# 0xPARC/plonkathon

Measured on AMD Instinct MI355X. Metric: proofs/sec at group_order=2^11 (PLONK prover hot path: NTT + quotient + KZG MSM), higher is better.
Workload: dtype u32x8 (254-bit Montgomery integers, BN254 Fr/Fq); 1 GPU; configs[1]: group_order=2^11, powersOfTau28_hez_final_11 SRS slice, synthetic squaring-chain witness, one distinct witness per proof; lockstep_batch=512, streams_per_gpu=20, parallelism=proof-sharded x1, ranks_in_communicator=1, gather_transport=none (single rank), msm_table_bytes=157571612672

## Files before the change

### plonkathon_amd/csrc/hip_compat.h

```cpp
#pragma once
#ifdef PLONK_EMU
#include "hip_emu.h"
#else
#include <hip/hip_runtime.h>
#define PLONK_HD __host__ __device__ __forceinline__
#define PLONK_HD_NOINLINE __host__ __device__ inline __attribute__((noinline))
#ifdef PLONK_FP_OUTLINE
#define PLONK_FP_CALL __host__ __device__ __attribute__((noinline))
#else
#define PLONK_FP_CALL __host__ __device__ __forceinline__
#endif
#define PLONK_DEV __device__ __forceinline__
#define PLONK_LAMBDA_INLINE __attribute__((always_inline))
#define PLONK_KERNEL(...) HIP_KERNEL_NAME(__VA_ARGS__)
#define PLONK_LAUNCH(kern, grid, block, shmem, stream, ...) \
    hipLaunchKernelGGL(kern, grid, block, shmem, stream, __VA_ARGS__)
#ifdef __HIP_DEVICE_COMPILE__
#define PLONK_SCHED_FENCE() __builtin_amdgcn_sched_barrier(0)
#else
#define PLONK_SCHED_FENCE() ((void)0)
#endif
#define PLONK_DYN_SMEM(name) extern __shared__ __attribute__((aligned(16))) unsigned char name[]
#endif

#ifndef PLONK_SHORT_KERNEL_PRIORITY
#define PLONK_SHORT_KERNEL_PRIORITY 3
#endif
#ifndef PLONK_WORK_KERNEL_PRIORITY
#define PLONK_WORK_KERNEL_PRIORITY 1
#endif
#if defined(__HIP_DEVICE_COMPILE__)
#define PLONK_SHORT_KERNEL() __builtin_amdgcn_s_setprio(PLONK_SHORT_KERNEL_PRIORITY)
#define PLONK_WORK_KERNEL() __builtin_amdgcn_s_setprio(PLONK_WORK_KERNEL_PRIORITY)
#else
#define PLONK_SHORT_KERNEL() ((void)0)
#define PLONK_WORK_KERNEL() ((void)0)
#endif

#ifndef PLONK_SMALL_FORMS
#define PLONK_SMALL_FORMS 23
#endif
#define PLONK_BESIDE_ACC(lanes, bit) PLONK_BESIDE_ACC_##bit(lanes)
#if (PLONK_SMALL_FORMS) & 1
#define PLONK_BESIDE_ACC_1(lanes) __launch_bounds__(lanes, 5)
#else
#define PLONK_BESIDE_ACC_1(lanes) __launch_bounds__(lanes)
#endif
#if (PLONK_SMALL_FORMS) & 2
#define PLONK_BESIDE_ACC_2(lanes) __launch_bounds__(lanes, 5)
#else
#define PLONK_BESIDE_ACC_2(lanes) __launch_bounds__(lanes)
#endif
#if (PLONK_SMALL_FORMS) & 4
#define PLONK_BESIDE_ACC_4(lanes) __launch_bounds__(lanes, 5)
#else
#define PLONK_BESIDE_ACC_4(lanes) __launch_bounds__(lanes)
#endif
#if (PLONK_SMALL_FORMS) & 16
#define PLONK_BESIDE_ACC_16(lanes) __launch_bounds__(lanes, 5)
#else
#define PLONK_BESIDE_ACC_16(lanes) __launch_bounds__(lanes)
#endif

#if defined(__HIP_DEVICE_COMPILE__)
#define PLONK_CHAIN_BEGIN() uint32_t plonk_chain_tok = 0
#define PLONK_CHAIN(acc) asm("" : "=s"(plonk_chain_tok) : "v"(acc), "0"(plonk_chain_tok))
#define PLONK_CHAIN_END(word) asm("" : "+v"(word) : "s"(plonk_chain_tok))
#else
#define PLONK_CHAIN_BEGIN() ((void)0)
#define PLONK_CHAIN(acc) ((void)0)
#define PLONK_CHAIN_END(word) ((void)0)
#endif
```

### plonkathon_amd/csrc/msm_comb.h

```cpp
#pragma once
#include <utility>

#include "msm_common.h"

#define MSM_COMB_MAX_TEETH 24
#define MSM_COMB_SEG_BITS 8
#define MSM_COMB_SCALAR_BITS 254
#define MSM_COMB_REDO 0x80000000u
PLONK_HD bool msm_comb_needs_redo(uint32_t v) { return (v & MSM_COMB_REDO) != 0 || v > MSM_DEFER_CAP; }

#define MSM_COMB_SKIP 0xffffffffu
struct alignas(16) MsmCombDigit4 { uint32_t d[4]; };

PLONK_HD unsigned msm_comb_columns(unsigned h) { return (MSM_COMB_SCALAR_BITS + h - 1) / h; }

struct MsmCombShape {
    unsigned h, a;
    unsigned top_bits, top_g;
    unsigned top_b;
    uint32_t top_entries;
};
PLONK_HD constexpr MsmCombShape msm_comb_shape(unsigned h, bool top) {
    MsmCombShape s{h, (MSM_COMB_SCALAR_BITS + h - 1) / h, 0, 0, 0, 0};
    if (!top) return s;
// ... 466 lines not shown
    ok &= g1l_wave_reduce_step<2>(acc, lane);
    ok &= g1l_wave_reduce_step<1>(acc, lane);
    if (!ok) atomicOr(n_deferred + m, MSM_COMB_REDO);
    if (lane == 0) colsum[m * a + j] = g1l_to_piece_wide(acc);
}

template <unsigned LPM> __global__ void PLONK_BESIDE_ACC(64, 1) msm_comb_finalize_kernel(const G1Xyzz* sums, size_t M, unsigned G, unsigned a,
                                                                                       const G1Affine* lookup, unsigned hb, size_t n,
                                                                                       const MsmDeferred* deferred, size_t deferred_stride,
                                                                                       uint32_t* n_deferred, uint32_t* redo, Fq* out_xy, uint8_t* flags,
                                                                                       unsigned n_real, unsigned top_delta) {
    PLONK_SHORT_KERNEL();
    const size_t gid = (size_t)blockIdx.x * 64 + threadIdx.x, m = gid / LPM;
    const unsigned l = (unsigned)(gid % LPM), lane = threadIdx.x;
    G1XyzzL acc = g1l_identity();
    bool ok = true;
    bool listed = false;
    if (m < M && l < a) {
        const uint32_t seen = n_deferred[m];
        listed = l == 0 && msm_comb_needs_redo(seen);
        const uint32_t nd = msm_comb_needs_redo(seen) ? 0u : seen;
        const unsigned jtop = l + ((a - 1 - l) / LPM) * LPM;
#pragma unroll 1
        for (int j = (int)jtop; j >= 0; j -= (int)LPM) {
            if (j != (int)jtop)
#pragma unroll 1
                for (unsigned d = 0; d < LPM; d++) g1l_dbl(acc);
#pragma unroll 1
            for (unsigned g = 0; g < G; g++) ok &= g1l_add_fast<true>(acc, g1l_from_piece(&sums[(m * G + g) * a + j]));
#pragma unroll 1
            for (uint32_t k = 0; k < nd; k++) {
                const MsmDeferred e = deferred[m * deferred_stride + k];
                if (e.bucket / n != (uint32_t)j || e.entry == MSM_COMB_SKIP) continue;
                const size_t i = e.bucket - (size_t)j * n;
                const G1Affine* src = lookup + ((msm_comb_block_of(i, n_real, top_delta) << hb) + (e.entry & 0x7fffffffu));
                const Fq x = fp_load(&src->x), y = fp_load(&src->y);
                if (!(fp_is_zero(x) && fp_is_zero(y))) ok &= g1l_madd_fast(acc, x, y, (e.entry >> 31) != 0);
            }
        }
#pragma unroll 1
        for (unsigned d = 0; d < l; d++) g1l_dbl(acc);
    }
    if constexpr (LPM >= 2) ok &= g1l_wave_reduce_step<1, true>(acc, lane);
    if constexpr (LPM >= 4) ok &= g1l_wave_reduce_step<2, true>(acc, lane);
    if constexpr (LPM >= 8) ok &= g1l_wave_reduce_step<4, true>(acc, lane);
    if constexpr (LPM >= 16) ok &= g1l_wave_reduce_step<8, true>(acc, lane);
    if constexpr (LPM >= 32) ok &= g1l_wave_reduce_step<16, true>(acc, lane);
    if constexpr (LPM >= 64) ok &= g1l_wave_reduce_step<32, true>(acc, lane);
    if (m < M && !ok && !msm_comb_needs_redo(atomicOr(n_deferred + m, MSM_COMB_REDO))) listed = true;
    if (listed) msm_redo_append(redo, (uint32_t)m, (uint32_t)M);
    if (m < M && l == 0) msm_store_result(g1l_to_xyzz(acc), m, out_xy, flags);
}

__global__ void __launch_bounds__(256) msm_comb_slow_kernel(const G1Affine* lookup, unsigned hb, unsigned a, const uint32_t* digits, size_t n, size_t rs,
                                                            size_t is, const uint32_t* redo, unsigned M, Fq* out_xy, uint8_t* flags, unsigned n_real,
                                                            unsigned top_delta) {
    PLONK_SHORT_KERNEL();
    __shared__ G1Xyzz red[256];
    const unsigned tid = threadIdx.x, count = redo[0] < M ? redo[0] : M;
#pragma unroll 1
    for (unsigned k = blockIdx.x; k < count; k += gridDim.x) {
        const unsigned m = redo[1 + k];
        if (m >= M) continue;
        const uint32_t* dg = digits + (size_t)m * a * rs;
        G1Xyzz acc = g1_xyzz_identity();
#pragma unroll 1
        for (int j = (int)a - 1; j >= 0; j--) {
            g1_dbl(acc);
#pragma unroll 1
            for (size_t i = tid; i < n; i += 256) {
                const uint32_t d = dg[(size_t)j * rs + i * is];
                if (d == MSM_COMB_SKIP) continue;
                const G1Affine* src = lookup + ((msm_comb_block_of(i, n_real, top_delta) << hb) + (d & 0x7fffffffu));
                G1Affine pt;
                pt.x = fp_load(&src->x);
                pt.y = fp_load(&src->y);
                if (d >> 31) pt.y = fp_neg(pt.y);
                g1_madd<true>(acc, pt);
            }
        }
        msm_fold_store(red, acc, tid, 256, m, out_xy, flags);
        __syncthreads();
    }
}

PLONK_DEV bool msm_comb_entry_matches(const G1Affine& P0, const MsmCombScale& k, unsigned a, unsigned h, uint32_t idx, const G1Affine* e) {
    const G1Affine P = g1_to_affine(msm_comb_scaled_base(P0, k));
    const G1Xyzz v = msm_comb_entry_slow(P, a, h, idx);
    const Fq ex = fp_load(&e->x), ey = fp_load(&e->y);
    if (g1_is_identity(v)) return fp_is_zero(ex) && fp_is_zero(ey);
    return fp_eq(fp_mul(ex, v.zz), v.x) && fp_eq(fp_mul(ey, v.zzz), v.y);
}
__global__ void __launch_bounds__(64) msm_comb_verify_kernel(const G1Affine* bases, const G1Affine* lookup, size_t n, unsigned a, unsigned h,
                                                             unsigned samples, MsmCombScale k, unsigned* mismatches) {
    const size_t t = (size_t)blockIdx.x * blockDim.x + threadIdx.x;
    if (t >= n + 2 * (size_t)samples) return;
    const uint32_t mask = (1u << (h - 1)) - 1u;
    size_t i;
    uint32_t idx;
    if (t < n) {
        i = t;
        idx = mask;
    } else {
        const unsigned s = (unsigned)(t - n) >> 1;
        i = n <= samples ? (s < n ? s : n - 1) : (size_t)s * (n - 1) / (samples - 1);
        idx = ((t - n) & 1) ? (0x55555555u & mask) : 0u;
    }
    G1Affine b;
    b.x = fp_load(&bases[i].x);
    b.y = fp_load(&bases[i].y);
    if (!msm_comb_entry_matches(b, k, a, h, idx, lookup + ((i << (h - 1)) + idx))) atomicAdd(mismatches, 1u);
}

__global__ void __launch_bounds__(64) msm_comb_verify_top_kernel(const G1Affine* bases, const G1Affine* lookup, size_t n, unsigned a, unsigned h, unsigned g,
                                                                 unsigned B, MsmCombScale k, unsigned* mismatches) {
    const size_t grp = (size_t)blockIdx.x * blockDim.x + threadIdx.x;
    if (grp >= msm_comb_top_groups(n, g)) return;
    const unsigned L = a * h, j = (unsigned)(grp % a);
    G1Xyzz sum = g1_xyzz_identity();
    uint32_t idx = 0, pw = 1;
#pragma unroll 1
    for (unsigned pos = 0; pos < g; pos++, pw *= B) {
        const size_t i = grp * g + pos;
        idx += ((B - 1) / 2 + (i < n ? 1u : 0u)) * pw;
        if (i >= n) continue;
        G1Affine b;
        b.x = fp_load(&bases[i].x);
        b.y = fp_load(&bases[i].y);
        G1Xyzz p = msm_comb_scaled_base(b, k);
#pragma unroll 1
        for (unsigned d = 0; d < L - j; d++) g1_dbl(p);
// ... 237 lines not shown
```

### plonkathon_amd/csrc/prover.hip

```cpp
#include <assert.h>
#include <string.h>

#include <array>
#include <vector>

#include "prover.h"
#include "g1_codec.h"
#include "prover_scans.h"
#include "prover_intake.h"
#include "prover_blind.h"

__global__ void pi_coeffs_kernel(const Fr* pub, size_t l, const Fr* roots_inv, size_t n, size_t B, Fr n_inv, Fr* pic) {
    PLONK_SHORT_KERNEL();
    const size_t total = B * n;
    for (size_t gI = (size_t)blockIdx.x * blockDim.x + threadIdx.x; gI < total; gI += (size_t)gridDim.x * blockDim.x) {
        const size_t b = gI / n, j = gI - b * n;
        Fr acc = fp_zero<FrParams>();
        for (size_t i = 0; i < l; i++) acc = fp_add(acc, fp_mul(fp_load(pub + b * l + i), fp_load(roots_inv + ((i * j) & (n - 1)))));
        fp_store(pic + gI, fp_neg(fp_mul(acc, n_inv)));
    }
}
__global__ void pi_coset_kernel(const Fr* pub, size_t l, const Fr* li_big, size_t n4, size_t B, Fr* pi_big) {
    PLONK_SHORT_KERNEL();
    const size_t total = B * n4;
    for (size_t gI = (size_t)blockIdx.x * blockDim.x + threadIdx.x; gI < total; gI += (size_t)gridDim.x * blockDim.x) {
        const size_t b = gI / n4, k = gI - b * n4;
        Fr acc = fp_zero<FrParams>();
        for (size_t i = 0; i < l; i++) acc = fp_add(acc, fp_mul(fp_load(pub + b * l + i), fp_load(li_big + i * n4 + k)));
        fp_store(pi_big + gI, fp_neg(acc));
    }
}
struct Zh4 { Fr v[4]; };
__global__ void li_coset_kernel(const Fr* xs, const Fr* roots, size_t n4, size_t n, size_t l, Zh4 zh, Fr n_inv, Fr* li) {
    const size_t total = l * n4;
    for (size_t gI = (size_t)blockIdx.x * blockDim.x + threadIdx.x; gI < total; gI += (size_t)gridDim.x * blockDim.x) {
        const size_t i = gI / n4, k = gI - i * n4;
        const Fr wi = fp_load(roots + i);
        const Fr num = fp_mul(fp_mul(wi, n_inv), zh.v[k / n]);
        fp_store(li + gI, fp_mul(num, fp_inv(fp_sub(fp_load(xs + k), wi))));
    }
}

__global__ void __launch_bounds__(2 * TC_LANES) transcript_kernel(int round, ProofState* st, size_t B, const Fq* commit_xy,
                                                                  const uint8_t* flags, ChallengeConsts cc) {
    PLONK_SHORT_KERNEL();
    __shared__ TcShared shared[2];
    const unsigned grp = threadIdx.x / TC_LANES, lane = threadIdx.x % TC_LANES;
    TcShared& sh = shared[grp];
    size_t b = (size_t)blockIdx.x * 2 + grp;
    const bool live = b < B;
    if (!live) b = B - 1;
    ProofState& s = st[b];
    TcState t = tc_load(s.transcript, lane);
    uint32_t error = 0;
    Fr c0 = fp_zero<FrParams>(), c1 = fp_zero<FrParams>();

    if (round >= 1 && round <= 3) {
        const unsigned first_slot = round == 1 ? 0 : round == 2 ? 3 : 4, count = round == 2 ? 1 : 3;
        if (lane < 2 * count) {
            const size_t slot = (size_t)first_slot + lane / 2;
            const uint8_t fl = flags[slot * B + b];
            Fq v = fp_load(commit_xy + 2 * (slot * B + b) + (lane & 1));
            if (fl) {
                v = fp_zero<FqParams>();
                error = 1;
            }
            limbs_to_be32(v.v, sh.msg + 32 * lane);
        }
    } else if (round == 4 && lane < PROOF_EVALS) {
        Fr e = fp_from_mont(s.evals[lane]);
        limbs_to_be32(e.v, sh.msg + 32 * lane);
    }
    __syncthreads();
    tc_round(t, sh, lane, cc, round, c0, c1);
    if (!live) return;
    tc_store(t, lane, s.transcript);
    if (error) s.error = 1;
    if (lane == 0) {
        if (round == 0) s.error = 0;
        if (round == 1) { s.beta = c0; s.gamma = c1; }
        if (round == 2) { s.alpha = c0; s.fft_cofactor = c1; }
        if (round == 3) s.zeta = c0;
        if (round == 4) s.v = c0;
    }
}

struct ZhInv { Fr v[4]; };
struct QuotientIn { const Fr* wit[5]; const Fr* fixed[FX_COUNT]; const Fr* l0; const Fr* xs; const uint32_t* cid; unsigned fixed_stride; };
__global__ void __launch_bounds__(256) quotient_kernel(QuotientIn in, ZhInv zh, const ProofState* st, RoundChallenges direct, unsigned n4, Fr* quot,
                                                       unsigned coset_log, unsigned out_stride) {
    PLONK_WORK_KERNEL();
    typedef FpL<FrParams> L;
    const unsigned b = blockIdx.y;
    const L beta = fpl_from_fp_uniform(st ? st[b].beta : direct.beta), gamma = fpl_from_fp_uniform(st ? st[b].gamma : direct.gamma),
            alpha = fpl_from_fp_uniform(st ? st[b].alpha : direct.alpha);
    const L one = fpl_one<FrParams>();
    const size_t row = (size_t)b * n4;
    const size_t fx = in.cid ? (size_t)in.cid[b] * in.fixed_stride : 0;
    for (unsigned k = blockIdx.x * blockDim.x + threadIdx.x; k < n4; k += gridDim.x * blockDim.x) {
        const unsigned cr = coset_log ? k >> coset_log : 0u, cmask = coset_log ? (1u << coset_log) - 1u : 0u;
        const unsigned kw = coset_log ? ((k & ~cmask) | ((k + 1) & cmask))
                                      : ((k + 4 < n4) ? k + 4 : k + 4 - n4);
        const auto ld = [&](const Fr* p) PLONK_LAMBDA_INLINE { return fpl_from_fp(fp_load(p)); };
        const L a = ld(in.wit[0] + row + k), bb = ld(in.wit[1] + row + k), c = ld(in.wit[2] + row + k);
        const L t1 = fpl_mul_add(a, ld(in.fixed[FX_QL] + fx + k), bb, ld(in.fixed[FX_QR] + fx + k));
        const L ab = fpl_mul(a, bb);
        const L t2 = fpl_mul_add(ab, ld(in.fixed[FX_QM] + fx + k), c, ld(in.fixed[FX_QO] + fx + k));
        const L gate = fpl_norm(fpl_add(fpl_add(t1, t2), fpl_add(ld(in.wit[3] + row + k), ld(in.fixed[FX_QC] + fx + k))));
        const L bx = fpl_mul(beta, ld(in.xs + k));
        const L u1 = fpl_norm(fpl_add(gamma, bx));
        const L u2 = fpl_norm(fpl_add(u1, bx));
        const L u3 = fpl_norm(fpl_add(u2, bx));
        const L z = ld(in.wit[4] + row + k);
        L p1 = fpl_mul(fpl_add(a, u1), z);
        p1 = fpl_mul(fpl_add(bb, u2), p1);
        p1 = fpl_mul(fpl_add(c, u3), p1);
        const L v1 = fpl_norm(fpl_add(gamma, fpl_mul(beta, ld(in.fixed[FX_S1] + fx + k))));
        L p2 = fpl_mul(fpl_add(a, v1), ld(in.wit[4] + row + kw));
        const L v2 = fpl_norm(fpl_add(gamma, fpl_mul(beta, ld(in.fixed[FX_S2] + fx + k))));
        p2 = fpl_mul(fpl_add(bb, v2), p2);
        const L v3 = fpl_norm(fpl_add(gamma, fpl_mul(beta, ld(in.fixed[FX_S3] + fx + k))));
        p2 = fpl_mul(fpl_add(c, v3), p2);
        const L first = fpl_mul(fpl_sub(z, one), ld(in.l0 + k));
        const L inner = fpl_add(fpl_sub(p1, p2), fpl_mul(alpha, first));
        const L acc = fpl_add(gate, fpl_mul(alpha, inner));
        L zhi;
        if (coset_log >= 6) zhi = fpl_from_fp_uniform(zh.v[cr]);
        else zhi = fpl_from_fp(zh.v[coset_log ? cr : (k & 3)]);
        fp_store(quot + (size_t)b * out_stride + k, fpl_pack_canonical(fpl_mul(acc, zhi)));
    }
}

__global__ void quotient_combine_kernel(Fr* quot, size_t n, size_t stride, size_t B, Fr ci, Fr g1_inv, Fr g2_inv_half, Fr half) {
    PLONK_SHORT_KERNEL();
    const size_t total = B * n;
    for (size_t gI = (size_t)blockIdx.x * blockDim.x + threadIdx.x; gI < total; gI += (size_t)gridDim.x * blockDim.x) {
        const size_t b = gI / n, i = gI - b * n;
        Fr* q = quot + b * stride + i;
        const Fr h0 = fp_load(q), h1 = fp_load(q + n), h2 = fp_load(q + 2 * n);
        const Fr s1 = fp_sub(h0, h2), p = fp_add(h0, h2);
        const Fr m = fp_sub(fp_dbl(h1), fp_mul(ci, s1));
        fp_store(q, fp_mul(fp_add(p, m), half));
// ... 161 lines not shown
static size_t batch_n_vectors(const plonk_prover* p) { return 17 + 5 * p->circuit.qcosets; }
static std::array<BatchBuffer, 14> batch_buffers(plonk_prover* p) {
    plonk_prover::Rounds& r = p->rounds;
    plonk_prover::Results& o = p->results;
    const size_t e = sizeof(Fr);
    return {{{(void**)&r.wit_lag, STAGED_N_VECTORS, 0, 0, true}, {(void**)&r.z_lag, 1}, {(void**)&r.coef, 5}, {(void**)&r.big, 5 * p->circuit.qcosets}, {(void**)&r.quot, 4},
             {(void**)&r.num, 1}, {(void**)&r.wz, 2}, {(void**)&r.closes, 0, 2 * sizeof(uint32_t)}, {(void**)&r.lin_w, 0, sizeof(LinWeights)}, {(void**)&r.blind, 0, sizeof(BlindState)},
             {(void**)&o.commit_xy, 0, PROOF_POINTS * 2 * sizeof(Fq)}, {(void**)&o.commit_flags, 0, PROOF_POINTS},
             {(void**)&o.state, 0, sizeof(ProofState)}, {(void**)&p->intake.pub, 0, p->circuit.n_public * e, e, true}}};
}

static void free_batch(plonk_prover* p, bool rounds_only = false) {
    for (const BatchBuffer& b : batch_buffers(p))
        if (!(rounds_only && b.in_set)) dev_free_all({b.slot});
    dev_free_all({(void**)&p->rounds.seg});
    p->rounds.seg_cap = p->intake.resident_b = p->rounds.cap_b = 0;
    if (rounds_only) return;
    dev_free_all({(void**)&p->intake.vars.buf});
    p->intake.vars.cap = p->intake.cap_b = 0;
}

static int ensure_segments(plonk_prover* p, size_t B) {
    const size_t need = scan_scratch_elems(B, prover_segments(p, B));
    return dev_grow(p->circuit.ctx->stream, &p->rounds.seg_cap, need, {{(void**)&p->rounds.seg, need * sizeof(Fr)}});
}

static int ensure_buffers(plonk_prover* p, size_t B, bool rounds_only) {
    if (B <= p->rounds.cap_b && (rounds_only || B <= p->intake.cap_b)) return ensure_segments(p, B);
    PLONK_CHECK_HIP(hipStreamSynchronize(p->circuit.ctx->stream));
    free_batch(p, rounds_only);
    int rc = PLONK_OK;
    size_t vectors = 0;
    for (const BatchBuffer& b : batch_buffers(p)) {
        if (rc == PLONK_OK && !(rounds_only && b.in_set)) rc = dev_alloc(b.slot, B * (b.n_vectors * p->circuit.n * sizeof(Fr) + b.bytes) + b.extra);
        vectors += b.n_vectors;
    }
    assert(vectors == batch_n_vectors(p));
    if (rc != PLONK_OK) {
        free_batch(p, rounds_only);
        if (rc == PLONK_ERR_NOMEM)
            plonk_set_error("a batch of %zu proofs of group_order %zu needs %zu bytes of device memory", B, p->circuit.n,
                            batch_n_vectors(p) * B * p->circuit.n * sizeof(Fr));
        return rc;
    }
    p->rounds.cap_b = B;
    if (!rounds_only) p->intake.cap_b = B;
    return ensure_segments(p, B);
}
static int ensure_batch(plonk_prover* p, size_t B) { return ensure_buffers(p, B, false); }
static int ensure_rounds(plonk_prover* p, size_t B) { return ensure_buffers(p, B, true); }

static void transcript_round(plonk_prover* p, size_t B, int round) {
    PLONK_LAUNCH(transcript_kernel, dim3((unsigned)((B + 1) / 2)), dim3(2 * TC_LANES), 0, p->circuit.ctx->stream, round, p->results.state, B,
                 (const Fq*)p->results.commit_xy, (const uint8_t*)p->results.commit_flags, p->circuit.chal);
}

static int commit(plonk_prover* p, size_t B, const Fr* lag, const Fr* coef, size_t count, size_t first_point) {
    const plonk_prover::Circuit& c = p->circuit;
    return msm_run_device(c.ctx, p->lag_srs ? p->lag_srs : c.srs, p->lag_srs ? lag : coef, c.n, count * B, c.n, p->results.commit_xy + 2 * first_point * B,
                          p->results.commit_flags + first_point * B);
}

static void blind_commit(plonk_prover* p, size_t B, unsigned first_point, unsigned count) {
    PLONK_LAUNCH(blind_commit_kernel, dim3((unsigned)B, count), dim3(BLIND_LANES), 0, p->circuit.ctx->stream, (const BlindState*)p->rounds.blind,
                 (const G1Affine*)p->blinding_src.htab, first_point, B, p->results.commit_xy, p->results.commit_flags);
}

static int blinders_for_run(plonk_prover* p, size_t B) {
    plonk_prover::Blinding& bl = p->blinding_src;
    hipStream_t s = p->circuit.ctx->stream;
    PLONK_REQUIRE(!bl.explicit_batch || bl.explicit_batch == B, PLONK_ERR_STATE, "run: batch %zu, but the blinders were set for a batch of %zu", B,
                  bl.explicit_batch);
    PLONK_REQUIRE(bl.explicit_batch || bl.seeded, PLONK_ERR_STATE,
                  "run: batch %zu is to be blinded, but neither plonk_prover_set_blinders nor plonk_prover_seed_blinders has been called", B);
    if (bl.explicit_batch) {
        PLONK_LAUNCH(blind_load_kernel, grid1(B * BLIND_COUNT), dim3(256), 0, s, (const Fr*)bl.explicit_b, B, p->rounds.blind);
        bl.explicit_batch = 0;
    } else {
        BlindSeed in;
        memcpy(in.seed, bl.seed, 32);
        in.run = bl.runs;
        PLONK_LAUNCH(blind_derive_kernel, dim3((unsigned)((B + 1) / 2)), dim3(2 * TC_LANES), 0, s, in, B, p->circuit.chal, p->rounds.blind);
    }
    bl.runs++;
    return PLONK_OK;
}

static int prover_init(plonk_prover* p, plonk_ctx* ctx, plonk_srs* srs, unsigned log_n, unsigned K, const uint8_t* selectors_le32, const size_t* n_public);

static int prover_create(plonk_ctx* ctx, plonk_srs* srs, unsigned log_n, unsigned K, const uint8_t* selectors_le32, const size_t* n_public, plonk_prover** out) {
    PLONK_ENTER(ctx);
    PLONK_REQUIRE(log_n >= 1 && log_n + 2 <= PLONK_FR_TWO_ADICITY, PLONK_ERR_ARG, "group_order 2^%u out of range", log_n);
    const size_t n = (size_t)1 << log_n;
    PLONK_REQUIRE(log_n <= PROVER_MAX_LOG_N, PLONK_ERR_ARG, "the batched prover supports group_order <= %u (got %zu)", 1u << PROVER_MAX_LOG_N, n);
    PLONK_REQUIRE(srs->n_points >= n, PLONK_ERR_ARG, "SRS has %zu powers, group_order is %zu", srs->n_points, n);
    for (unsigned c = 0; c < K; c++) PLONK_REQUIRE(n_public[c] <= n, PLONK_ERR_ARG, "more public inputs than rows");
    plonk_prover* p = new plonk_prover();
    memset((void*)p, 0, sizeof *p);
    const int rc = prover_init(p, ctx, srs, log_n, K, selectors_le32, n_public);
    if (rc != PLONK_OK) {
        plonk_prover_destroy(p);
        return rc;
    }
    *out = p;
    return PLONK_OK;
}

// ... 144 lines not shown
    PLONK_ENTER(p->circuit.ctx);
    const unsigned seg = (flags & PLONK_PROVER_SEGMENTS_MASK) >> 8;
    PLONK_REQUIRE(seg <= 9 && (!seg || (p->circuit.n >> (seg - 1)) >= 16), PLONK_ERR_ARG,
                  "2^%u segments: at most 256, of at least 16 rows each (group_order %zu)", seg ? seg - 1 : 0, p->circuit.n);
    const unsigned form = (flags & PLONK_PROVER_SOLVE_FORM_MASK) >> 16;
    PLONK_REQUIRE(form <= PLONK_PROVER_SOLVE_LEVELS, PLONK_ERR_ARG, "solve form %u: 0 (automatic), 1 (one lane per proof) or 2 (levels)", form);
    const bool blinding = (flags & PLONK_PROVER_BLINDING) != 0;
    if (blinding != p->blinding) PLONK_TRY(set_blinding(p, blinding));
    p->seg_forced = seg;
    p->solve_forced = form;
    p->lag_srs = nullptr;
    if (flags & PLONK_PROVER_LAGRANGE_COMMITS) PLONK_TRY(msm_lagrange_srs(p->circuit.ctx, p->circuit.srs, p->circuit.log_n, &p->lag_srs));
    return PLONK_OK;
}

int plonk_prover_destroy(plonk_prover* p) {
    if (!p) return PLONK_OK;
    plonk_prover::Circuit& c = p->circuit;
    if (c.ctx) {
        plonk_use_device(c.ctx->device);
        hipStreamSynchronize(c.ctx->stream);
        if (c.ctx->copy_stream) hipStreamSynchronize(c.ctx->copy_stream);
    }
    free_batch(p);
    free_coset_tables(c);
    dev_free_all({(void**)&c.fixed_lag, (void**)&c.fixed_coef, (void**)&p->blinding_src.htab, (void**)&p->blinding_src.explicit_b});
    intake_destroy(p);
    free(c.n_public_of);
    delete p;
    return PLONK_OK;
}

int plonk_prover_run(plonk_prover* p, size_t B) {
    PLONK_REQUIRE(p && B, PLONK_ERR_ARG, "bad argument");
    PLONK_REQUIRE(B == p->intake.resident_b, PLONK_ERR_STATE, "run: batch %zu, but %zu witnesses are resident", B, p->intake.resident_b);
    const plonk_prover::Circuit& c = p->circuit;
    const plonk_prover::Rounds& r = p->rounds;
    PLONK_ENTER(c.ctx);
    plonk_ctx* ctx = c.ctx;
    const size_t n = c.n, n4 = 4 * n;
    const unsigned log_n = c.log_n;
    hipStream_t s = ctx->stream;
    const Fr* pub = p->intake.pub;
    ProofState* state = p->results.state;
    PLONK_REQUIRE(B <= 65535, PLONK_ERR_ARG, "batch %zu exceeds 65535 (the proofs are a grid's second dimension)", B);
    PLONK_TRY(ensure_segments(p, B));
    const unsigned S = prover_segments(p, B);
    const bool blind = p->blinding;
    BlindState* bs = r.blind;
    if (blind) PLONK_TRY(blinders_for_run(p, B));
    const uint32_t* cid = c.n_circuits > 1 ? p->labels.dev : nullptr;

    transcript_round(p, B, 0);
    PLONK_CHECK_HIP(hipMemsetAsync(r.closes + B, 0, B * sizeof(uint32_t), s));
    PLONK_LAUNCH(gate_check_kernel, grid1(B * n), dim3(256), 0, s, (const Fr*)r.wit_lag, pub, c.n_public,
                 c.sparse_pi ? (const Fr*)nullptr : (const Fr*)(r.wit_lag + 3 * B * n), (const Fr*)c.fixed_lag, cid, n, B, r.closes + B);
    if (c.sparse_pi) {
        PLONK_TRY(ntt_run(ctx, ntt_inverse(r.wit_lag, r.coef, log_n, 3 * B)));
        if (c.n_public) PLONK_LAUNCH(pi_coeffs_kernel, grid1(B * n), dim3(256), 0, s, pub, c.n_public, c.roots_inv, n, B, c.n_inv, r.coef + 3 * B * n);
        else PLONK_CHECK_HIP(hipMemsetAsync(r.coef + 3 * B * n, 0, B * n * sizeof(Fr), s));
    } else {
        PLONK_TRY(ntt_run(ctx, ntt_inverse(r.wit_lag, r.coef, log_n, 4 * B)));
    }
    PLONK_TRY(commit(p, B, r.wit_lag, r.coef, 3, 0));
    if (blind) blind_commit(p, B, 0, 3);
    transcript_round(p, B, 1);
    GrandProductIn gp = {};
    for (int k = 0; k < 3; k++) {
        gp.abc[k] = r.wit_lag + (size_t)k * B * n;
        gp.sig[k] = c.fixed_lag + (FX_S1 + k) * n;
    }
    gp.cid = cid;
    gp.sig_stride = FX_COUNT * n;
    PLONK_TRY(prof_begin(ctx, "prover_grand_product", 11.0 * 32.0 * (double)n * (double)B));
    PLONK_TRY(scan_grand_product(s, S, gp, c.roots, state, RoundChallenges{}, n, B, r.z_lag, r.closes, r.num, r.wz, r.seg));
    PLONK_TRY(prof_end(ctx));
    PLONK_TRY(ntt_run(ctx, ntt_inverse(r.z_lag, r.coef + 4 * B * n, log_n, B)));
    PLONK_TRY(commit(p, B, r.z_lag, r.coef + 4 * B * n, 1, 3));
    if (blind) blind_commit(p, B, 3, 1);
    transcript_round(p, B, 2);
    const size_t n3 = c.qcosets * n;
    if (c.sparse_pi) {
        PLONK_TRY(ntt_run(ctx, coset_call(c, r.coef, r.big, 3 * B)));
        PLONK_TRY(ntt_run(ctx, coset_call(c, r.coef + 4 * B * n, r.big + 4 * B * n3, B)));
        if (c.n_public) PLONK_LAUNCH(pi_coset_kernel, grid1(B * n3), dim3(256), 0, s, pub, c.n_public, (const Fr*)c.li_big, n3, B, r.big + 3 * B * n3);
        else PLONK_CHECK_HIP(hipMemsetAsync(r.big + 3 * B * n3, 0, B * n3 * sizeof(Fr), s));
    } else {
        PLONK_TRY(ntt_run(ctx, coset_call(c, r.coef, r.big, 5 * B)));
    }
    if (blind) {
        BlindZh bz;
        for (int k = 0; k < 4; k++) bz.v[k] = c.zh[k];
        PLONK_LAUNCH(blind_coset_kernel, grid1(B * n3), dim3(256), 0, s, (const BlindState*)bs, (const Fr*)c.x_big, bz, log_n, B, r.big);
    }
    ZhInv zh;
    for (int k = 0; k < 4; k++) zh.v[k] = c.zh_inv[k < (int)c.qcosets ? k : 0];
    QuotientIn qi = {};
    for (int k = 0; k < 5; k++) qi.wit[k] = r.big + (size_t)k * B * n3;
    for (int k = 0; k < FX_COUNT; k++) qi.fixed[k] = c.fixed_big + (size_t)k * n3;
    qi.l0 = c.l0_big;
    qi.xs = c.x_big;
    qi.cid = cid;
    qi.fixed_stride = (unsigned)(FX_COUNT * n3);
    PLONK_LAUNCH(quotient_kernel, dim3((unsigned)((n3 + 255) / 256), (unsigned)B), dim3(256), 0, s, qi, zh, (const ProofState*)state, RoundChallenges{},
                 (unsigned)n3, r.quot, log_n, (unsigned)n4);
    NttCall back{r.quot, r.quot, log_n, true, B};
    back.in_bstride = back.out_bstride = n4;
// ... 199 lines not shown
```

### plonkathon_amd/csrc/prover_scans.h

```cpp
#pragma once
#include "prover.h"

#define SCAN_THREADS 256

struct LaneRange { size_t lo, hi, per; };
PLONK_DEV LaneRange block_lane_range(size_t n, unsigned tid) {
    LaneRange r;
    r.per = (n + SCAN_THREADS - 1) / SCAN_THREADS;
    r.lo = tid * r.per;
    r.hi = (r.lo + r.per < n) ? r.lo + r.per : n;
    return r;
}
PLONK_DEV LaneRange seg_lane_range(size_t n, unsigned S, unsigned seg, unsigned tid) {
    const size_t L = n / S, per = (L + SCAN_THREADS - 1) / SCAN_THREADS, s_lo = (size_t)seg * L, s_hi = s_lo + L;
    LaneRange r;
    r.per = per;
    r.lo = s_lo + (size_t)tid * per < s_hi ? s_lo + (size_t)tid * per : s_hi;
    r.hi = r.lo + per < s_hi ? r.lo + per : s_hi;
    return r;
}

struct GrandProductIn { const Fr* abc[3]; const Fr* sig[3]; const uint32_t* cid; size_t sig_stride; };
struct GpProducts { Fr n, d; };

PLONK_DEV GpProducts gp_chunk_factors(const GrandProductIn& in, const Fr* roots, const Fr& beta, const Fr& gamma, size_t b, size_t n,
                                      const LaneRange& r, Fr* NUM, Fr* DEN) {
    const Fr *A = in.abc[0] + b * n, *Bv = in.abc[1] + b * n, *C = in.abc[2] + b * n;
    const size_t so = in.cid ? (size_t)in.cid[b] * in.sig_stride : 0;
    const Fr *S1 = in.sig[0] + so, *S2 = in.sig[1] + so, *S3 = in.sig[2] + so;
    const Fr one = fp_one<FrParams>();
    GpProducts p = {one, one};
    for (size_t i = r.lo; i < r.hi; i++) {
        Fr a = fp_load(A + i), bb = fp_load(Bv + i), c = fp_load(C + i);
        Fr bw = fp_mul(beta, fp_load(roots + i));
        Fr ag = fp_add(a, gamma), bg = fp_add(bb, gamma), cg = fp_add(c, gamma);
        Fr num = fp_mul(fp_mul(fp_add(ag, bw), fp_add(bg, fp_dbl(bw))), fp_add(cg, fp_mul3(bw)));
        Fr den = fp_mul(fp_mul(fp_add(ag, fp_mul(beta, fp_load(S1 + i))), fp_add(bg, fp_mul(beta, fp_load(S2 + i)))),
                        fp_add(cg, fp_mul(beta, fp_load(S3 + i))));
        if (fp_is_zero(den)) {
            num = fp_zero<FrParams>();
            den = one;
        }
        fp_store(NUM + i, num);
        fp_store(DEN + i, den);
        p.d = fp_mul(p.d, den);
        p.n = fp_mul(p.n, num);
    }
    return p;
}

PLONK_DEV void block_scan_products(Fr* sc_n, Fr* sc_d, unsigned tid) {
    for (unsigned off = 1; off < SCAN_THREADS; off <<= 1) {
        Fr vn = sc_n[tid], vd = sc_d[tid];
        if (tid >= off) vn = fp_mul(vn, sc_n[tid - off]);
        if (tid + off < SCAN_THREADS) vd = fp_mul(vd, sc_d[tid + off]);
        __syncthreads();
        sc_n[tid] = vn;
        sc_d[tid] = vd;
        __syncthreads();
    }
}

PLONK_DEV Fr gp_chunk_apply(const Fr* NUM, Fr* DEN, Fr* Z, const LaneRange& r, Fr run_n, Fr after_d, const Fr& tinv) {
    for (size_t k = r.hi; k-- > r.lo;) {
        after_d = fp_mul(after_d, fp_load(DEN + k));
        fp_store(DEN + k, after_d);
    }
    for (size_t i = r.lo; i < r.hi; i++) {
        fp_store(Z + i, fp_mul(fp_mul(run_n, fp_load(DEN + i)), tinv));
        run_n = fp_mul(run_n, fp_load(NUM + i));
    }
    return run_n;
}

__global__ void PLONK_BESIDE_ACC(SCAN_THREADS, 4) grand_product_kernel(GrandProductIn in, const Fr* roots, const ProofState* st,
                                                                     RoundChallenges direct, size_t n, Fr* z_out,
                                                                     uint32_t* closes, Fr* num_buf, Fr* den_buf) {
    PLONK_SHORT_KERNEL();
    __shared__ Fr sc_n[SCAN_THREADS], sc_d[SCAN_THREADS];
    __shared__ Fr tot_inv;
    const size_t b = blockIdx.x;
    const unsigned tid = threadIdx.x;
    const Fr beta = st ? st[b].beta : direct.beta, gamma = st ? st[b].gamma : direct.gamma;
    Fr *NUM = num_buf + b * n, *DEN = den_buf + b * n;
    const LaneRange r = block_lane_range(n, tid);
    const Fr one = fp_one<FrParams>();
    const GpProducts p = gp_chunk_factors(in, roots, beta, gamma, b, n, r, NUM, DEN);
    sc_n[tid] = p.n;
    sc_d[tid] = p.d;
    __syncthreads();
    block_scan_products(sc_n, sc_d, tid);
    if (tid == 0) tot_inv = fp_inv(sc_d[0]);
    __syncthreads();
    const Fr run_n = tid ? sc_n[tid - 1] : one;
    const Fr after_d = (tid + 1 < SCAN_THREADS) ? sc_d[tid + 1] : one;
    const Fr tinv = tot_inv;
    const Fr all_n = gp_chunk_apply(NUM, DEN, z_out + b * n, r, run_n, after_d, tinv);
    if (tid == SCAN_THREADS - 1) closes[b] = fp_eq(fp_mul(all_n, tinv), fp_one<FrParams>()) ? 1u : 0u;
}

PLONK_DEV void eval_chunk_sums(Fr (*red)[SCAN_THREADS], const Fr* coef, const Fr* fixed_coef, const uint32_t* cid, const Fr& zeta, const Fr& zeta_w,
                               size_t b, size_t n, size_t B, const LaneRange& r, unsigned tid) {
    if (cid) fixed_coef += (size_t)cid[b] * FX_COUNT * n;
    const Fr* polys[NEVAL] = {coef + (0 * B + b) * n, coef + (1 * B + b) * n, coef + (2 * B + b) * n,
                              fixed_coef + FX_S1 * n,  fixed_coef + FX_S2 * n,  coef + (4 * B + b) * n,
                              coef + (3 * B + b) * n};
    const Fr shift_z = fp_pow_u64(zeta, (uint64_t)r.lo), shift_zw = fp_pow_u64(zeta_w, (uint64_t)r.lo);
    typedef FpL<FrParams> L;
    const L zl = fpl_from_fp_uniform(zeta), zwl = fpl_from_fp_uniform(zeta_w);
    L acc[NEVAL];
    wave_for<NEVAL>([&](auto P_) { acc[decltype(P_)::value] = fpl_zero<FrParams>(); });
#pragma unroll 1
    for (size_t i = r.hi; i-- > r.lo;)
        wave_for<NEVAL>([&](auto P_) {
            constexpr unsigned p = decltype(P_)::value;
            acc[p] = fpl_add(fpl_mul(acc[p], p == 5 ? zwl : zl), fpl_from_fp(fp_load(polys[p] + i)));
        });
    const L sh_z = fpl_from_fp(shift_z), sh_zw = fpl_from_fp(shift_zw);
    wave_for<NEVAL>([&](auto P_) {
        constexpr unsigned p = decltype(P_)::value;
        red[p][tid] = r.lo < r.hi ? fpl_pack_canonical(fpl_mul(acc[p], p == 5 ? sh_zw : sh_z)) : fp_zero<FrParams>();
    });
    __syncthreads();
    for (unsigned s = SCAN_THREADS / 2; s > 0; s >>= 1) {
        if (tid < s)
            for (int p = 0; p < NEVAL; p++) red[p][tid] = fp_add(red[p][tid], red[p][tid + s]);
        __syncthreads();
    }
}

__global__ void __launch_bounds__(SCAN_THREADS) eval_kernel(const Fr* coef, const Fr* fixed_coef, const uint32_t* cid, Fr w, ProofState* st,
                                                            size_t n, size_t B) {
    PLONK_SHORT_KERNEL();
    __shared__ Fr red[NEVAL][SCAN_THREADS];
    const size_t b = blockIdx.x;
    const unsigned tid = threadIdx.x;
    const Fr zeta = st[b].zeta, zeta_w = fp_mul(zeta, w);
    eval_chunk_sums(red, coef, fixed_coef, cid, zeta, zeta_w, b, n, B, block_lane_range(n, tid), tid);
    if (tid < NEVAL) st[b].evals[tid] = red[tid][0];
}

PLONK_DEV Fr divide_point(const ProofState* st, size_t b, const Fr& w, int which) {
    Fr x0 = st[b].zeta;
    if (which) x0 = fp_mul(x0, w);
    return x0;
}
PLONK_DEV Fr divide_chunk_horner(const Fr* p, const LaneRange& r, const Fr& x0) {
    Fr h = fp_zero<FrParams>();
    for (size_t i = r.hi; i-- > r.lo;) h = fp_add(fp_mul(h, x0), fp_load(p + i));
    return h;
}
PLONK_DEV void block_suffix_scan_affine(Fr* sc, unsigned tid, Fr m) {
    for (unsigned off = 1; off < SCAN_THREADS; off <<= 1) {
        Fr vv = sc[tid];
        if (tid + off < SCAN_THREADS) vv = fp_add(vv, fp_mul(m, sc[tid + off]));
        __syncthreads();
        sc[tid] = vv;
        m = fp_sqr(m);
        __syncthreads();
    }
}
PLONK_DEV void divide_chunk_writeback(const Fr* p, Fr* out, const LaneRange& r, const Fr& x0, Fr q) {
    for (size_t i = r.hi; i-- > r.lo;) {
        fp_store(out + i, q);
        q = fp_add(fp_load(p + i), fp_mul(x0, q));
    }
}

__global__ void __launch_bounds__(SCAN_THREADS) divide_linear_kernel(const Fr* p_in, size_t in_stride, int which,
                                                                     Fr w, const ProofState* st, size_t n, Fr* q_out) {
    PLONK_SHORT_KERNEL();
    __shared__ Fr sc[SCAN_THREADS];
    const size_t b = blockIdx.x;
    const unsigned tid = threadIdx.x;
    const Fr x0 = divide_point(st, b, w, which);
    const Fr* p = p_in + b * in_stride;
    const LaneRange r = block_lane_range(n, tid);
    sc[tid] = divide_chunk_horner(p, r, x0);
    __syncthreads();
    block_suffix_scan_affine(sc, tid, fp_pow_u64(x0, (uint64_t)r.per));
    divide_chunk_writeback(p, q_out + b * n, r, x0, (tid + 1 < SCAN_THREADS) ? sc[tid + 1] : fp_zero<FrParams>());
}


__global__ void __launch_bounds__(SCAN_THREADS) gp_seg_factors_kernel(GrandProductIn in, const Fr* roots, const ProofState* st,
                                                                      RoundChallenges direct, size_t n, Fr* num_buf, Fr* den_buf,
                                                                      Fr* seg_n, Fr* seg_d) {
    PLONK_SHORT_KERNEL();
    __shared__ Fr sc_n[SCAN_THREADS], sc_d[SCAN_THREADS];
    const size_t b = blockIdx.y;
    const unsigned tid = threadIdx.x, S = gridDim.x;
    const Fr beta = st ? st[b].beta : direct.beta, gamma = st ? st[b].gamma : direct.gamma;
// ... 10 lines not shown
    }
    if (tid == 0) {
        fp_store(seg_n + b * S + blockIdx.x, sc_n[0]);
        fp_store(seg_d + b * S + blockIdx.x, sc_d[0]);
    }
}

__global__ void __launch_bounds__(SCAN_THREADS) gp_seg_carries_kernel(unsigned S, Fr* seg_n, Fr* seg_d, Fr* tot_inv, uint32_t* closes) {
    PLONK_SHORT_KERNEL();
    __shared__ Fr sc_n[SCAN_THREADS], sc_d[SCAN_THREADS];
    const size_t b = blockIdx.x;
    const unsigned tid = threadIdx.x;
    const Fr one = fp_one<FrParams>();
    sc_n[tid] = tid < S ? fp_load(seg_n + b * S + tid) : one;
    sc_d[tid] = tid < S ? fp_load(seg_d + b * S + tid) : one;
    __syncthreads();
    block_scan_products(sc_n, sc_d, tid);
    if (tid < S) {
        fp_store(seg_n + b * S + tid, tid ? sc_n[tid - 1] : one);
        fp_store(seg_d + b * S + tid, tid + 1 < SCAN_THREADS ? sc_d[tid + 1] : one);
    }
    if (tid == 0) {
        const Fr tinv = fp_inv(sc_d[0]);
        fp_store(tot_inv + b, tinv);
        closes[b] = fp_eq(fp_mul(sc_n[SCAN_THREADS - 1], tinv), one) ? 1u : 0u;
    }
}

__global__ void __launch_bounds__(SCAN_THREADS) gp_seg_apply_kernel(size_t n, const Fr* seg_n, const Fr* seg_d, const Fr* tot_inv,
                                                                    const Fr* num_buf, Fr* den_buf, Fr* z_out) {
    PLONK_SHORT_KERNEL();
    __shared__ Fr sc_n[SCAN_THREADS], sc_d[SCAN_THREADS];
    const size_t b = blockIdx.y;
    const unsigned tid = threadIdx.x, S = gridDim.x;
    const Fr* NUM = num_buf + b * n;
    Fr* DEN = den_buf + b * n;
    const LaneRange r = seg_lane_range(n, S, blockIdx.x, tid);
    const Fr one = fp_one<FrParams>();
    Fr pn = one, pd = one;
    for (size_t i = r.lo; i < r.hi; i++) {
        pn = fp_mul(pn, fp_load(NUM + i));
        pd = fp_mul(pd, fp_load(DEN + i));
    }
    sc_n[tid] = pn;
    sc_d[tid] = pd;
    __syncthreads();
    block_scan_products(sc_n, sc_d, tid);
    Fr run_n = fp_load(seg_n + b * S + blockIdx.x), after_d = fp_load(seg_d + b * S + blockIdx.x);
    if (tid) run_n = fp_mul(run_n, sc_n[tid - 1]);
    if (tid + 1 < SCAN_THREADS) after_d = fp_mul(after_d, sc_d[tid + 1]);
    gp_chunk_apply(NUM, DEN, z_out + b * n, r, run_n, after_d, fp_load(tot_inv + b));
}

__global__ void __launch_bounds__(SCAN_THREADS) eval_seg_kernel(const Fr* coef, const Fr* fixed_coef, const uint32_t* cid, Fr w, const ProofState* st,
                                                                size_t n, size_t B, Fr* part) {
    PLONK_SHORT_KERNEL();
    __shared__ Fr red[NEVAL][SCAN_THREADS];
    const size_t b = blockIdx.y;
    const unsigned tid = threadIdx.x, S = gridDim.x;
    const Fr zeta = st[b].zeta, zeta_w = fp_mul(zeta, w);
    eval_chunk_sums(red, coef, fixed_coef, cid, zeta, zeta_w, b, n, B, seg_lane_range(n, S, blockIdx.x, tid), tid);
    if (tid < NEVAL) fp_store(part + (b * S + blockIdx.x) * NEVAL + tid, red[tid][0]);
}

__global__ void __launch_bounds__(SCAN_THREADS) eval_seg_finish_kernel(const Fr* part, unsigned S, ProofState* st) {
    PLONK_SHORT_KERNEL();
    __shared__ Fr red[SCAN_THREADS];
    const size_t b = blockIdx.x;
    const unsigned tid = threadIdx.x, p = tid / 32, l = tid % 32;
    Fr acc = fp_zero<FrParams>();
    if (p < NEVAL)
        for (unsigned s = l; s < S; s += 32) acc = fp_add(acc, fp_load(part + (b * S + s) * NEVAL + p));
    red[tid] = acc;
    __syncthreads();
    for (unsigned s = 16; s > 0; s >>= 1) {
        if (l < s) red[tid] = fp_add(red[tid], red[tid + s]);
        __syncthreads();
    }
    if (l == 0 && p < NEVAL) st[b].evals[p] = red[tid];
}

struct DivideIn { const Fr* p_in[2]; Fr* q_out[2]; };
__global__ void __launch_bounds__(SCAN_THREADS) divide_seg_horner_kernel(DivideIn in, Fr w, const ProofState* st, size_t n, Fr* seg_h) {
    PLONK_SHORT_KERNEL();
    __shared__ Fr sc[SCAN_THREADS];
    const size_t b = blockIdx.y, B = gridDim.y;
    const unsigned tid = threadIdx.x, S = gridDim.x, z = blockIdx.z;
    const Fr x0 = divide_point(st, b, w, z);
    const LaneRange r = seg_lane_range(n, S, blockIdx.x, tid);
    sc[tid] = divide_chunk_horner(in.p_in[z] + b * n, r, x0);
    __syncthreads();
    Fr m = fp_pow_u64(x0, (uint64_t)r.per);
    for (unsigned off = 1; off < SCAN_THREADS; off <<= 1) {
        if ((tid & (2 * off - 1)) == 0) sc[tid] = fp_add(sc[tid], fp_mul(m, sc[tid + off]));
        m = fp_sqr(m);
        __syncthreads();
    }
    if (tid == 0) fp_store(seg_h + ((size_t)z * B + b) * S + blockIdx.x, sc[0]);
}

__global__ void __launch_bounds__(SCAN_THREADS) divide_seg_carries_kernel(unsigned S, Fr w, const ProofState* st, size_t n, Fr* seg_h) {
    PLONK_SHORT_KERNEL();
    __shared__ Fr sc[SCAN_THREADS];
    const size_t b = blockIdx.x, B = gridDim.x;
    const unsigned tid = threadIdx.x, z = blockIdx.z;
    const Fr x0 = divide_point(st, b, w, z);
    Fr* h = seg_h + ((size_t)z * B + b) * S;
    sc[tid] = tid < S ? fp_load(h + tid) : fp_zero<FrParams>();
    __syncthreads();
    block_suffix_scan_affine(sc, tid, fp_pow_u64(x0, (uint64_t)(n / S)));
    if (tid < S) fp_store(h + tid, tid + 1 < SCAN_THREADS ? sc[tid + 1] : fp_zero<FrParams>());
}

__global__ void __launch_bounds__(SCAN_THREADS) divide_seg_apply_kernel(DivideIn in, Fr w, const ProofState* st, size_t n, const Fr* seg_h) {
    PLONK_SHORT_KERNEL();
// ... 89 lines not shown
```

Baseline: 52250 proofs/s.

## Add occupancy hints, wave-shuffle eval reductions, fold gate-fail reset into transcript

Adds min-blocks launch-bound hints to the quotient, eval and slow MSM kernels through new PLONK_SMALL_FORMS bits. The evaluation reduction now splits the polynomials into three register-lighter passes and sums with wave shuffles, replacing the large shared-memory tree reduction that needed a barrier per step. The slow MSM kernel switches g1_madd to its false template variant. The gate-fail buffer is now zeroed inside the round-0 transcript kernel, removing a separate memset. Forcing occupancy can cause register spills, and the madd flag change may alter edge-case handling.

```diff
diff --git a/plonkathon_amd/csrc/hip_compat.h b/plonkathon_amd/csrc/hip_compat.h
--- a/plonkathon_amd/csrc/hip_compat.h
+++ b/plonkathon_amd/csrc/hip_compat.h
@@ -38,7 +38,7 @@
 #endif
 
 #ifndef PLONK_SMALL_FORMS
-#define PLONK_SMALL_FORMS 23
+#define PLONK_SMALL_FORMS 127
 #endif
 #define PLONK_BESIDE_ACC(lanes, bit) PLONK_BESIDE_ACC_##bit(lanes)
 #if (PLONK_SMALL_FORMS) & 1
@@ -61,6 +61,21 @@
 #else
 #define PLONK_BESIDE_ACC_16(lanes) __launch_bounds__(lanes)
 #endif
+#if (PLONK_SMALL_FORMS) & 8
+#define PLONK_BESIDE_ACC_8(lanes) __launch_bounds__(lanes, 5)
+#else
+#define PLONK_BESIDE_ACC_8(lanes) __launch_bounds__(lanes)
+#endif
+#if (PLONK_SMALL_FORMS) & 32
+#define PLONK_BESIDE_ACC_32(lanes) __launch_bounds__(lanes, 5)
+#else
+#define PLONK_BESIDE_ACC_32(lanes) __launch_bounds__(lanes)
+#endif
+#if (PLONK_SMALL_FORMS) & 64
+#define PLONK_BESIDE_ACC_64(lanes) __launch_bounds__(lanes, 5)
+#else
+#define PLONK_BESIDE_ACC_64(lanes) __launch_bounds__(lanes)
+#endif
 
 #if defined(__HIP_DEVICE_COMPILE__)
 #define PLONK_CHAIN_BEGIN() uint32_t plonk_chain_tok = 0
diff --git a/plonkathon_amd/csrc/msm_comb.h b/plonkathon_amd/csrc/msm_comb.h
--- a/plonkathon_amd/csrc/msm_comb.h
+++ b/plonkathon_amd/csrc/msm_comb.h
@@ -542,7 +542,7 @@
     if (m < M && l == 0) msm_store_result(g1l_to_xyzz(acc), m, out_xy, flags);
 }
 
-__global__ void __launch_bounds__(256) msm_comb_slow_kernel(const G1Affine* lookup, unsigned hb, unsigned a, const uint32_t* digits, size_t n, size_t rs,
+__global__ void PLONK_BESIDE_ACC(256, 32) msm_comb_slow_kernel(const G1Affine* lookup, unsigned hb, unsigned a, const uint32_t* digits, size_t n, size_t rs,
                                                             size_t is, const uint32_t* redo, unsigned M, Fq* out_xy, uint8_t* flags, unsigned n_real,
                                                             unsigned top_delta) {
     PLONK_SHORT_KERNEL();
@@ -566,7 +566,7 @@
                 pt.x = fp_load(&src->x);
                 pt.y = fp_load(&src->y);
                 if (d >> 31) pt.y = fp_neg(pt.y);
-                g1_madd<true>(acc, pt);
+                g1_madd<false>(acc, pt);
             }
         }
         msm_fold_store(red, acc, tid, 256, m, out_xy, flags);
diff --git a/plonkathon_amd/csrc/prover.hip b/plonkathon_amd/csrc/prover.hip
--- a/plonkathon_amd/csrc/prover.hip
+++ b/plonkathon_amd/csrc/prover.hip
@@ -42,7 +42,7 @@
 }
 
 __global__ void __launch_bounds__(2 * TC_LANES) transcript_kernel(int round, ProofState* st, size_t B, const Fq* commit_xy,
-                                                                  const uint8_t* flags, ChallengeConsts cc) {
+                                                                  const uint8_t* flags, ChallengeConsts cc, uint32_t* gate_fail) {
     PLONK_SHORT_KERNEL();
     __shared__ TcShared shared[2];
     const unsigned grp = threadIdx.x / TC_LANES, lane = threadIdx.x % TC_LANES;
@@ -77,7 +77,10 @@
     tc_store(t, lane, s.transcript);
     if (error) s.error = 1;
     if (lane == 0) {
-        if (round == 0) s.error = 0;
+        if (round == 0) {
+            s.error = 0;
+            gate_fail[b] = 0;
+        }
         if (round == 1) { s.beta = c0; s.gamma = c1; }
         if (round == 2) { s.alpha = c0; s.fft_cofactor = c1; }
         if (round == 3) s.zeta = c0;
@@ -87,7 +90,7 @@
 
 struct ZhInv { Fr v[4]; };
 struct QuotientIn { const Fr* wit[5]; const Fr* fixed[FX_COUNT]; const Fr* l0; const Fr* xs; const uint32_t* cid; unsigned fixed_stride; };
-__global__ void __launch_bounds__(256) quotient_kernel(QuotientIn in, ZhInv zh, const ProofState* st, RoundChallenges direct, unsigned n4, Fr* quot,
+__global__ void PLONK_BESIDE_ACC(256, 64) quotient_kernel(QuotientIn in, ZhInv zh, const ProofState* st, RoundChallenges direct, unsigned n4, Fr* quot,
                                                        unsigned coset_log, unsigned out_stride) {
     PLONK_WORK_KERNEL();
     typedef FpL<FrParams> L;
@@ -355,7 +358,7 @@
 
 static void transcript_round(plonk_prover* p, size_t B, int round) {
     PLONK_LAUNCH(transcript_kernel, dim3((unsigned)((B + 1) / 2)), dim3(2 * TC_LANES), 0, p->circuit.ctx->stream, round, p->results.state, B,
-                 (const Fq*)p->results.commit_xy, (const uint8_t*)p->results.commit_flags, p->circuit.chal);
+                 (const Fq*)p->results.commit_xy, (const uint8_t*)p->results.commit_flags, p->circuit.chal, p->rounds.closes + B);
 }
 
 static int commit(plonk_prover* p, size_t B, const Fr* lag, const Fr* coef, size_t count, size_t first_point) {
@@ -606,7 +609,6 @@
     const uint32_t* cid = c.n_circuits > 1 ? p->labels.dev : nullptr;
 
     transcript_round(p, B, 0);
-    PLONK_CHECK_HIP(hipMemsetAsync(r.closes + B, 0, B * sizeof(uint32_t), s));
     PLONK_LAUNCH(gate_check_kernel, grid1(B * n), dim3(256), 0, s, (const Fr*)r.wit_lag, pub, c.n_public,
                  c.sparse_pi ? (const Fr*)nullptr : (const Fr*)(r.wit_lag + 3 * B * n), (const Fr*)c.fixed_lag, cid, n, B, r.closes + B);
     if (c.sparse_pi) {
diff --git a/plonkathon_amd/csrc/prover_scans.h b/plonkathon_amd/csrc/prover_scans.h
--- a/plonkathon_amd/csrc/prover_scans.h
+++ b/plonkathon_amd/csrc/prover_scans.h
@@ -1,5 +1,6 @@
 #pragma once
 #include "prover.h"
+#include "wave.h"
 
 #define SCAN_THREADS 256
 
@@ -99,45 +100,77 @@
     if (tid == SCAN_THREADS - 1) closes[b] = fp_eq(fp_mul(all_n, tinv), fp_one<FrParams>()) ? 1u : 0u;
 }
 
-PLONK_DEV void eval_chunk_sums(Fr (*red)[SCAN_THREADS], const Fr* coef, const Fr* fixed_coef, const uint32_t* cid, const Fr& zeta, const Fr& zeta_w,
-                               size_t b, size_t n, size_t B, const LaneRange& r, unsigned tid) {
-    if (cid) fixed_coef += (size_t)cid[b] * FX_COUNT * n;
-    const Fr* polys[NEVAL] = {coef + (0 * B + b) * n, coef + (1 * B + b) * n, coef + (2 * B + b) * n,
-                              fixed_coef + FX_S1 * n,  fixed_coef + FX_S2 * n,  coef + (4 * B + b) * n,
-                              coef + (3 * B + b) * n};
-    const Fr shift_z = fp_pow_u64(zeta, (uint64_t)r.lo), shift_zw = fp_pow_u64(zeta_w, (uint64_t)r.lo);
+#define EVAL_WAVES (SCAN_THREADS / 64)
+struct EvalWaveSums { Fr v[EVAL_WAVES][NEVAL]; };
+
+PLONK_DEV Fr fr_wave_sum(Fr v, unsigned lane) {
+    const auto step = [&](auto M_) PLONK_LAMBDA_INLINE {
+        constexpr unsigned MASK = decltype(M_)::value;
+        Fr o;
+#pragma unroll
+        for (int i = 0; i < 8; i++) o.v[i] = wave_lane_xor<MASK>(v.v[i], lane);
+        v = fp_add(v, o);
+    };
+    step(WaveIdx<32>{});
+    step(WaveIdx<16>{});
+    step(WaveIdx<8>{});
+    step(WaveIdx<4>{});
+    step(WaveIdx<2>{});
+    step(WaveIdx<1>{});
+    return v;
+}
+
+template <unsigned K0, unsigned NK>
+PLONK_DEV void eval_pass(EvalWaveSums& ws, const Fr* const (&polys)[NEVAL], const unsigned (&slot)[NEVAL], const FpL<FrParams>& xl, const Fr& shift,
+                         const LaneRange& r, unsigned tid) {
     typedef FpL<FrParams> L;
-    const L zl = fpl_from_fp_uniform(zeta), zwl = fpl_from_fp_uniform(zeta_w);
-    L acc[NEVAL];
-    wave_for<NEVAL>([&](auto P_) { acc[decltype(P_)::value] = fpl_zero<FrParams>(); });
+    L acc[NK];
+    wave_for<NK>([&](auto K_) { acc[decltype(K_)::value] = fpl_zero<FrParams>(); });
 #pragma unroll 1
     for (size_t i = r.hi; i-- > r.lo;)
-        wave_for<NEVAL>([&](auto P_) {
-            constexpr unsigned p = decltype(P_)::value;
-            acc[p] = fpl_add(fpl_mul(acc[p], p == 5 ? zwl : zl), fpl_from_fp(fp_load(polys[p] + i)));
+        wave_for<NK>([&](auto K_) {
+            constexpr unsigned k = decltype(K_)::value;
+            acc[k] = fpl_add(fpl_mul(acc[k], xl), fpl_from_fp(fp_load(polys[K0 + k] + i)));
         });
-    const L sh_z = fpl_from_fp(shift_z), sh_zw = fpl_from_fp(shift_zw);
-    wave_for<NEVAL>([&](auto P_) {
-        constexpr unsigned p = decltype(P_)::value;
-        red[p][tid] = r.lo < r.hi ? fpl_pack_canonical(fpl_mul(acc[p], p == 5 ? sh_zw : sh_z)) : fp_zero<FrParams>();
+    const L sh = fpl_from_fp(shift);
+    const unsigned wave = tid / 64, lane = tid % 64;
+    wave_for<NK>([&](auto K_) {
+        constexpr unsigned k = decltype(K_)::value;
+        const Fr mine = r.lo < r.hi ? fpl_pack_canonical(fpl_mul(acc[k], sh)) : fp_zero<FrParams>();
+        const Fr sum = fr_wave_sum(mine, lane);
+        if (lane == 0) ws.v[wave][slot[K0 + k]] = sum;
     });
-    __syncthreads();
-    for (unsigned s = SCAN_THREADS / 2; s > 0; s >>= 1) {
-        if (tid < s)
-            for (int p = 0; p < NEVAL; p++) red[p][tid] = fp_add(red[p][tid], red[p][tid + s]);
-        __syncthreads();
-    }
-}
-
-__global__ void __launch_bounds__(SCAN_THREADS) eval_kernel(const Fr* coef, const Fr* fixed_coef, const uint32_t* cid, Fr w, ProofState* st,
+    PLONK_SCHED_FENCE();
+}
+
+PLONK_DEV Fr eval_chunk_sums(EvalWaveSums& ws, const Fr* coef, const Fr* fixed_coef, const uint32_t* cid, const Fr& zeta, const Fr& zeta_w,
+                             size_t b, size_t n, size_t B, const LaneRange& r, unsigned tid) {
+    if (cid) fixed_coef += (size_t)cid[b] * FX_COUNT * n;
+    const Fr* const polys[NEVAL] = {coef + (4 * B + b) * n, coef + (0 * B + b) * n, coef + (1 * B + b) * n, coef + (2 * B + b) * n,
+                                    fixed_coef + FX_S1 * n,  fixed_coef + FX_S2 * n,  coef + (3 * B + b) * n};
+    const unsigned slot[NEVAL] = {5, 0, 1, 2, 3, 4, 6};
+    const Fr shift_z = fp_pow_u64(zeta, (uint64_t)r.lo), shift_zw = fp_pow_u64(zeta_w, (uint64_t)r.lo);
+    eval_pass<0, 1>(ws, polys, slot, fpl_from_fp_uniform(zeta_w), shift_zw, r, tid);
+    eval_pass<1, 3>(ws, polys, slot, fpl_from_fp_uniform(zeta), shift_z, r, tid);
+    eval_pass<4, 3>(ws, polys, slot, fpl_from_fp_uniform(zeta), shift_z, r, tid);
+    __syncthreads();
+    Fr total = fp_zero<FrParams>();
+    if (tid < NEVAL) {
+        total = ws.v[0][tid];
+        for (unsigned wv = 1; wv < EVAL_WAVES; wv++) total = fp_add(total, ws.v[wv][tid]);
+    }
+    return total;
+}
+
+__global__ void PLONK_BESIDE_ACC(SCAN_THREADS, 8) eval_kernel(const Fr* coef, const Fr* fixed_coef, const uint32_t* cid, Fr w, ProofState* st,
                                                             size_t n, size_t B) {
     PLONK_SHORT_KERNEL();
-    __shared__ Fr red[NEVAL][SCAN_THREADS];
+    __shared__ EvalWaveSums ws;
     const size_t b = blockIdx.x;
     const unsigned tid = threadIdx.x;
     const Fr zeta = st[b].zeta, zeta_w = fp_mul(zeta, w);
-    eval_chunk_sums(red, coef, fixed_coef, cid, zeta, zeta_w, b, n, B, block_lane_range(n, tid), tid);
-    if (tid < NEVAL) st[b].evals[tid] = red[tid][0];
+    const Fr total = eval_chunk_sums(ws, coef, fixed_coef, cid, zeta, zeta_w, b, n, B, block_lane_range(n, tid), tid);
+    if (tid < NEVAL) st[b].evals[tid] = total;
 }
 
 PLONK_DEV Fr divide_point(const ProofState* st, size_t b, const Fr& w, int which) {
@@ -254,15 +287,15 @@
     gp_chunk_apply(NUM, DEN, z_out + b * n, r, run_n, after_d, fp_load(tot_inv + b));
 }
 
-__global__ void __launch_bounds__(SCAN_THREADS) eval_seg_kernel(const Fr* coef, const Fr* fixed_coef, const uint32_t* cid, Fr w, const ProofState* st,
+__global__ void PLONK_BESIDE_ACC(SCAN_THREADS, 8) eval_seg_kernel(const Fr* coef, const Fr* fixed_coef, const uint32_t* cid, Fr w, const ProofState* st,
                                                                 size_t n, size_t B, Fr* part) {
     PLONK_SHORT_KERNEL();
-    __shared__ Fr red[NEVAL][SCAN_THREADS];
+    __shared__ EvalWaveSums ws;
     const size_t b = blockIdx.y;
     const unsigned tid = threadIdx.x, S = gridDim.x;
     const Fr zeta = st[b].zeta, zeta_w = fp_mul(zeta, w);
-    eval_chunk_sums(red, coef, fixed_coef, cid, zeta, zeta_w, b, n, B, seg_lane_range(n, S, blockIdx.x, tid), tid);
-    if (tid < NEVAL) fp_store(part + (b * S + blockIdx.x) * NEVAL + tid, red[tid][0]);
+    const Fr total = eval_chunk_sums(ws, coef, fixed_coef, cid, zeta, zeta_w, b, n, B, seg_lane_range(n, S, blockIdx.x, tid), tid);
+    if (tid < NEVAL) fp_store(part + (b * S + blockIdx.x) * NEVAL + tid, total);
 }
 
 __global__ void __launch_bounds__(SCAN_THREADS) eval_seg_finish_kernel(const Fr* part, unsigned S, ProofState* st) {
```

Result: faster. 52920 proofs/s (median of 6 runs) (+1.3%).
